# theouterlimitz/Audio-Mastering-Engine

Measured on NVIDIA B200. Metric: audio-sec mastered/sec (x realtime), higher is better.
Workload: dtype f64

## Files before the change

### audio_mastering_engine_b200/csrc/ame.cu

```cuda
#include <algorithm>
#include <cmath>
#include <cstdarg>
#include <cstdio>
#include <cstring>
#include <dlfcn.h>
#include <mutex>
#include <string>
#include <vector>

#include "ame_kernels.cuh"

using namespace ame;

namespace {

thread_local std::string g_err;

int fail(int code, const char *fmt, ...) {
    char buf[512];
    va_list ap;
    va_start(ap, fmt);
    vsnprintf(buf, sizeof buf, fmt, ap);
    va_end(ap);
    g_err = buf;
// ... 129 lines not shown
    int *d_meter_sp = nullptr;
    unsigned *d_meter_tp = nullptr;
    ame_loudness *d_loud_out = nullptr;
    ame_loudness *d_loud_any = nullptr;
    cudaStream_t s_in = nullptr, s_out = nullptr;
    std::vector<cudaEvent_t> ev_in, ev_run;
    std::vector<cudaEvent_t> ev_meter;
    bool timing = false;
    int t_step = -1, t_wave = 0;
    std::vector<cudaEvent_t> t_ev;
    std::vector<char> t_used;
    std::vector<cudaEvent_t> tl_ev;
    int tl_waves = 0;
};

namespace {

inline bool t_on(const ame_plan *p) {
    return p->timing && p->t_step >= 0 && p->t_step < kMaxTimedSteps && p->t_wave < kMaxTimedWaves;
}
inline size_t t_slot(const ame_plan *p, int kernel) {
    return ((size_t)p->t_step * kMaxTimedWaves + p->t_wave) * AME_N_KERNELS + kernel;
}
inline void t_begin(ame_plan *p, int kernel, cudaStream_t s) {
    if (t_on(p)) cudaEventRecord(p->t_ev[t_slot(p, kernel) * 2], s);
}
inline void t_end(ame_plan *p, int kernel, cudaStream_t s) {
    if (t_on(p)) {
        cudaEventRecord(p->t_ev[t_slot(p, kernel) * 2 + 1], s);
        p->t_used[t_slot(p, kernel)] = 1;
    }
}

int plan_alloc(ame_plan *p, void **ptr, size_t bytes) {
    *ptr = nullptr;
    if (bytes == 0) return AME_OK;
    cudaError_t e = dev_alloc(ptr, bytes);
    if (e != cudaSuccess) {
        *ptr = nullptr;
        return fail(AME_E_NOMEM, "device allocation of %zu bytes failed: %s", bytes, cudaGetErrorString(e));
    }
    p->allocs.push_back(*ptr);
    return AME_OK;
}

int dmalloc(ame_plan *p, void **ptr, size_t bytes) {
    const int rc = plan_alloc(p, ptr, bytes);
    if (rc == AME_OK) p->ws_bytes += bytes;
    return rc;
}

template <class T>
int upload(ame_plan *p, T **dptr, const std::vector<T> &v) {
    if (int rc = plan_alloc(p, (void **)dptr, v.size() * sizeof(T))) return rc;
    if (!v.empty()) CU(cudaMemcpy(*dptr, v.data(), v.size() * sizeof(T), cudaMemcpyHostToDevice));
    return AME_OK;
}

#define LAUNCH_CHECK(p)                                                                            \
    do {                                                                                           \
        cudaError_t e_ = cudaGetLastError();                                                       \
        if (e_ != cudaSuccess) return fail(AME_E_CUDA, "kernel launch failed: %s (%s:%d)", cudaGetErrorString(e_), __FILE__, __LINE__); \
        ++(p)->launches;                                                                           \
    } while (0)

int check_warmth(const ame_plan *p) {
    for (int t = 0; t < p->n_tracks; ++t)
        if (p->tracks[t].flags & AME_F_WARMTH) {
            const int l = p->tracks[t].warm_lut;
            if (l < 0 || l >= p->n_luts) return fail(AME_E_INVALID, "track %d needs warmth table %d but %d are set", t, l, p->n_luts);
        }
    return AME_OK;
}

struct Bufs {
    const int16_t *in = nullptr;
    int16_t *pre = nullptr, *bands = nullptr, *out = nullptr;
    uint16_t *rms = nullptr, *list = nullptr;
    int *tile_cnt = nullptr, *n_flagged = nullptr;
    GrpRec *grp = nullptr;
    double *att = nullptr;
    int64_t *hist = nullptr;
    int16_t *norm = nullptr;
    long long *lim_last = nullptr;
    LimStore lim_in{}, lim_out{};
    int *lim_need = nullptr;
};

Bufs slot_bufs(ame_plan *p, const Wave &w, const int16_t *d_in, int16_t *d_out) {
    const Slot &sl = p->slots[w.slot];
    Bufs b;
    b.in = d_in; b.out = d_out;
    b.pre = sl.pre - 2 * w.frame_lo;
    b.bands = sl.bands; b.rms = sl.rms; b.list = sl.list; b.tile_cnt = sl.tile_cnt; b.n_flagged = sl.n_flagged;
    b.grp = sl.grp; b.att = sl.att;
    b.norm = sl.norm ? sl.norm - 2 * w.frame_lo : nullptr;
    b.lim_last = sl.lim_last; b.lim_in = sl.lim_in; b.lim_out = sl.lim_out; b.lim_need = sl.lim_need;
    b.hist = (int64_t *)p->d_hist;
    return b;
}

int run_eq(ame_plan *p, const Wave &w, const int16_t *d_in, int16_t *d_pre, cudaStream_t s) {
    if (!w.eq.n) return AME_OK;
    t_begin(p, S_EQ, s);
    if (p->precision == 1)
        k_eq_f32<<<(w.eq.n + 127) / 128, 128, 0, s>>>(p->d_eq_jobs + w.eq.lo, w.eq.n, p->d_tracks, p->d_luts, d_in, d_pre);
    else
        k_eq<<<(w.eq.n + kEqBlock - 1) / kEqBlock, kEqBlock, 0, s>>>(p->d_eq_jobs + w.eq.lo, w.eq.n, p->d_tracks, p->d_luts, d_in, d_pre);
    LAUNCH_CHECK(p);
    t_end(p, S_EQ, s);
    return AME_OK;
}

int run_split(ame_plan *p, const Wave &w, const int16_t *d_pre, int16_t *d_bands, cudaStream_t s) {
    if (!w.split.n) return AME_OK;
    t_begin(p, S_SPLIT, s);
    if (w.xover_uni)
        k_band_split<true><<<(w.split.n + 127) / 128, 128, 0, s>>>(w.xover, p->d_split_jobs + w.split.lo, w.split.n, p->d_tracks, p->d_mb_delta,
                                                                   d_pre, d_bands, p->mb_frames);
    else
        k_band_split<false><<<(w.split.n + 127) / 128, 128, 0, s>>>(w.xover, p->d_split_jobs + w.split.lo, w.split.n, p->d_tracks, p->d_mb_delta,
                                                                    d_pre, d_bands, p->mb_frames);
    LAUNCH_CHECK(p);
    t_end(p, S_SPLIT, s);
    return AME_OK;
}

int chain_lanes(const ame_plan *p, int n_chains) {
    if (p->chain_warps < 0) return 1;
    if (p->chain_warps > 0) return 32 * p->chain_warps;
    if (n_chains * 2 <= p->n_sm) return 256;
    return (n_chains >= p->n_sm && p->slots.size() > 1) ? 64 : 128;
}

int run_compress(ame_plan *p, const Wave &w, const Bufs &b, cudaStream_t s) {
    if (!w.chain.n) return AME_OK;
    t_begin(p, S_FLAG, s);
    int *tile_base = b.tile_cnt + std::max(p->slot_tiles, 1);
    k_window_flag<<<w.wf.n, kWfThreads, 0, s>>>(p->d_wf_jobs + w.wf.lo, b.bands, b.rms, b.tile_cnt, b.grp);
    LAUNCH_CHECK(p);
    k_tile_prefix<<<w.chain.n, kWfThreads, 0, s>>>(p->d_chain_jobs + w.chain.lo, b.tile_cnt, tile_base, b.n_flagged);
    LAUNCH_CHECK(p);
    k_compact<<<(w.wf.n + kWfThreads / 32 - 1) / (kWfThreads / 32), kWfThreads, 0, s>>>(p->d_wf_jobs + w.wf.lo, w.wf.n, b.rms, b.tile_cnt,
                                                                                          tile_base, b.list, b.grp);
    LAUNCH_CHECK(p);
    t_end(p, S_FLAG, s);
    t_begin(p, S_CHAIN, s);
    const int lanes = chain_lanes(p, w.chain.n);
    k_att_chain<<<w.chain.n, std::max(lanes, 32), 0, s>>>(p->d_chain_jobs + w.chain.lo, b.list, b.n_flagged, p->d_tables, b.att, p->mb_frames,
                                            lanes, p->d_chain_stats + 2 * (size_t)w.chain.lo);
    LAUNCH_CHECK(p);
    t_end(p, S_CHAIN, s);
    t_begin(p, S_APPLY, s);
    k_compress_apply<<<(unsigned)((w.seg_hi - w.seg_lo + 3) / 4), 128, 0, s>>>(p->d_mb_chunks + w.mb_chunks.lo, w.mb_chunks.n, w.seg_lo, w.seg_hi,
                                                                                b.bands, b.grp, b.att, b.pre, p->mb_frames);
    LAUNCH_CHECK(p);
    t_end(p, S_APPLY, s);
    return AME_OK;
}

int run_hist(ame_plan *p, const Wave &w, const int16_t *d_pre, int64_t *d_hist, cudaStream_t s) {
    const int nt = w.track_hi - w.track_lo;
    if (nt <= 0) return AME_OK;
    CU(cudaMemsetAsync(p->d_peak + w.track_lo, 0, (size_t)nt * 4, s));
    if (w.kw.n) {
        t_begin(p, S_KW, s);
        if (w.kw_uni)
            k_kweight_energy<true><<<(w.kw.n + 127) / 128, 128, 0, s>>>(w.kw_cfg, p->d_kw_jobs + w.kw.lo, w.kw.n, p->d_tracks, p->d_tdev, d_pre,
                                                                        p->d_energy, p->d_peak);
        else
            k_kweight_energy<false><<<(w.kw.n + 127) / 128, 128, 0, s>>>(w.kw_cfg, p->d_kw_jobs + w.kw.lo, w.kw.n, p->d_tracks, p->d_tdev, d_pre,
                                                                         p->d_energy, p->d_peak);
        LAUNCH_CHECK(p);
        t_end(p, S_KW, s);
    }
    t_begin(p, S_TAIL, s);
    k_tail_peak<<<nt, 128, 0, s>>>(p->d_tracks, p->d_tdev, w.track_lo, w.track_hi, d_pre, p->d_peak);
    LAUNCH_CHECK(p);
    t_end(p, S_TAIL, s);
    CU(cudaMemsetAsync(p->d_tp + w.track_lo, 0, (size_t)nt * 4, s));
    if (w.true_peak && w.gain.n) {
        t_begin(p, S_TP, s);
        k_true_peak<<<w.gain.n, 256, 0, s>>>(p->d_gain_jobs + w.gain.lo, p->d_tracks, d_pre, p->d_tp);
        LAUNCH_CHECK(p);
        t_end(p, S_TP, s);
    }
    t_begin(p, S_HIST, s);
    k_block_hist<<<nt, 256, 0, s>>>(p->d_tdev, w.track_lo, p->d_energy, (long long *)d_hist, p->d_hist_st);
    LAUNCH_CHECK(p);
    t_end(p, S_HIST, s);
    return AME_OK;
}

int run_apply(ame_plan *p, const Wave &w, const int16_t *d_pre, int16_t *d_out, const Bufs &b, cudaStream_t s) {
    int16_t *d_norm = b.norm;
    long long *lim_last = b.lim_last;
    if (!w.gain.n) return AME_OK;
    t_begin(p, S_GAIN, s);
    if (w.limiter) CU(cudaMemsetAsync(lim_last, 0xff, (size_t)w.lim.n * sizeof(long long), s));
    k_apply_gain<<<w.gain.n, 256, 0, s>>>(p->d_gain_jobs + w.gain.lo, p->d_results, p->d_tracks, p->d_tdev, d_pre, d_out, d_norm, lim_last);
    LAUNCH_CHECK(p);
    t_end(p, S_GAIN, s);
    if (w.limiter) {
        t_begin(p, S_LIM, s);
        const GainJob *gj = p->d_lim_jobs + w.lim.lo;
        constexpr int kLimRounds = 2;
        int cap = 64;
        while (cap < p->lim_keep + 2) cap *= 2;
        const size_t smem = lim_smem_bytes(cap);
        for (int round = 0; round <= kLimRounds; ++round) {
            if (round == 0) {
                k_limiter<<<w.lim.n, 256, smem, s>>>(gj, w.lim.n, lim_last, p->d_tracks, d_norm, d_out, b.lim_in, b.lim_out, b.lim_need, 0, cap, p->lim_guess);
                LAUNCH_CHECK(p);
            }
            k_limiter<<<w.lim.n, 32, smem, s>>>(gj, w.lim.n, lim_last, p->d_tracks, d_norm, d_out, b.lim_in, b.lim_out, b.lim_need, round, cap, p->lim_guess);
            LAUNCH_CHECK(p);
            k_lim_verify<<<(w.lim.n + 3) / 4, 128, 0, s>>>(gj, w.lim.n, p->d_tracks, b.lim_in, b.lim_out, b.lim_need,
                                                             p->d_lim_stats + round);
            LAUNCH_CHECK(p);
        }
        k_lim_fallback<<<w.lim.n, 32, smem, s>>>(gj, w.lim.n, p->d_tracks, d_norm, d_out, b.lim_in, b.lim_out, b.lim_need, cap);
        LAUNCH_CHECK(p);
        t_end(p, S_LIM, s);
    }
    return AME_OK;
}

int run_gain(ame_plan *p, const Wave &w, const int16_t *d_pre, const int64_t *d_hist, int16_t *d_out, const Bufs &b, cudaStream_t s) {
    const int nt = w.track_hi - w.track_lo;
    if (nt <= 0) return AME_OK;
    t_begin(p, S_FIN, s);
    k_finalize<<<nt, 128, 0, s>>>(p->d_tracks, w.track_lo, w.track_hi, (const long long *)d_hist, p->d_hist_st, p->d_peak,
                                             p->d_tp, p->d_results);
    LAUNCH_CHECK(p);
    t_end(p, S_FIN, s);
    return run_apply(p, w, d_pre, d_out, b, s);
}

int run_meter(ame_plan *p, const Wave &w, const int16_t *buf, ame_loudness *res, cudaStream_t s) {
    if (!w.meter_tracks.n) return AME_OK;
    const int nt = w.track_hi - w.track_lo;
    CU(cudaMemsetAsync(p->d_meter_sp + w.track_lo, 0, (size_t)nt * 4, s));
    CU(cudaMemsetAsync(p->d_meter_tp + w.track_lo, 0, (size_t)nt * 4, s));
    if (w.meter_kw.n) {
        if (w.kw_uni)
            k_kweight_energy<true><<<(w.meter_kw.n + 127) / 128, 128, 0, s>>>(w.kw_cfg, p->d_meter_kw + w.meter_kw.lo, w.meter_kw.n, p->d_tracks,
                                                                              p->d_meter_tdev, buf, p->d_meter_energy, p->d_meter_sp);
        else
            k_kweight_energy<false><<<(w.meter_kw.n + 127) / 128, 128, 0, s>>>(w.kw_cfg, p->d_meter_kw + w.meter_kw.lo, w.meter_kw.n, p->d_tracks,
                                                                               p->d_meter_tdev, buf, p->d_meter_energy, p->d_meter_sp);
        LAUNCH_CHECK(p);
    }
    if (w.meter_peak.n) {
        k_meter_peak<<<w.meter_peak.n, 256, 0, s>>>(p->d_meter_peak + w.meter_peak.lo, p->d_tracks, buf, p->d_meter_tp, p->d_meter_sp);
        LAUNCH_CHECK(p);
    }
    k_meter_finalize<<<w.meter_tracks.n, 256, 0, s>>>(p->d_meter_tracks + w.meter_tracks.lo, p->d_tracks, p->d_meter_tdev, p->d_meter_energy,
                                                      p->d_meter_sp, p->d_meter_tp, res);
    LAUNCH_CHECK(p);
    return AME_OK;
}

int run_measure(ame_plan *p, const Wave &w, const Bufs &b, cudaStream_t s) {
    int rc;
    if ((rc = run_eq(p, w, b.in, b.pre, s))) return rc;
    if ((rc = run_split(p, w, b.pre, b.bands, s))) return rc;
    if ((rc = run_compress(p, w, b, s))) return rc;
    return run_hist(p, w, b.pre, b.hist, s);
}

int run_chain_of_stages(ame_plan *p, const Wave &w, const Bufs &b, cudaStream_t s) {
    int rc = run_measure(p, w, b, s);
    if (rc) return rc;
    return run_gain(p, w, b.pre, b.hist, b.out, b, s);
}

int drain(ame_plan *p, int rc) {
    (void)p;
    if (rc != AME_OK) cudaDeviceSynchronize();
    return rc;
}

}

extern "C" {

int ame_abi_version(void) { return AME_ABI_VERSION; }
size_t ame_sizeof_track_params(void) { return sizeof(ame_track_params); }
size_t ame_sizeof_track_result(void) { return sizeof(ame_track_result); }
size_t ame_sizeof_plan_options(void) { return sizeof(ame_plan_options); }
size_t ame_sizeof_loudness(void) { return sizeof(ame_loudness); }
const char *ame_last_error(void) { return g_err.c_str(); }
const char *ame_kernel_name(int slot) { return (slot >= 0 && slot < AME_N_KERNELS) ? kKernelNames[slot] : ""; }

int ame_device_count(int *count) {
    if (!count) return fail(AME_E_INVALID, "count is NULL");
    *count = 0;
    CU(cudaGetDeviceCount(count));
    return AME_OK;
}

void ame_plan_destroy(ame_plan *p) {
    if (!p) return;
    DeviceGuard guard(p->device);
    cudaDeviceSynchronize();
    for (void *q : p->allocs) dev_free(q);
// ... 601 lines not shown
```

### audio_mastering_engine_b200/csrc/ame_kernels.cuh

```cuda
#pragma once
#include <cuda_runtime.h>
#include <stdint.h>
#include "ame_layout.h"

namespace ame {

constexpr unsigned kFull = 0xffffffffu;

__constant__ double c_hist_bounds[1001];
__constant__ double c_hist_energy[1000];

__device__ __forceinline__ uint4 ldg16(const uint4 *p) { return __ldg(p); }

__device__ __forceinline__ double bq_step(const ame_biquad &c, double &z0, double &z1, double x) {
    double y = fma(c.b0, x, z0);
    z0 = fma(-c.a1, y, fma(c.b1, x, z1));
    z1 = fma(-c.a2, y, c.b2 * x);
    return y;
}

__device__ __forceinline__ double i16_to_f64(int x) {
    return __hiloint2double(0x43300000, (int)(0x80000000u ^ (unsigned)x)) - 4503601774854144.0;
}

// ... 507 lines not shown
    int exp0;
    bool open;
    bool ok;
};

__device__ __forceinline__ void segsum_begin(SegSum &u, double start) {
    u.margin = 0x7fffffffffffffffLL; u.at_p = 0; u.lo = 0; u.hi = -1; u.p = 0;
    u.exp0 = (int)(__double_as_longlong(start) >> 52);
    u.open = true; u.ok = u.exp0 > 0;
}

template <bool DUAL>
__device__ __forceinline__ bool list_step8(const AttEntry *e, double *al, int64_t i, int64_t lim, bool avec, double &a, double &b,
                                           SegSum &u, double &max_m, double &sum_dec) {
    double o[8];
#pragma unroll
    for (int k = 0; k < 8; ++k) {
        if (!DUAL) { max_m = fmax(max_m, e[k].m); sum_dec += e[k].dec; }
        if (DUAL && u.open && i + k < lim) {
            const long long ib = __double_as_longlong(b), im = __double_as_longlong(e[k].m);
            if (ib > im) {
                u.margin = min(u.margin, ib - im);
                const long long id = __double_as_longlong(e[k].dec);
                if (id != 0) {
                    const int ed = (int)(id >> 52);
                    const long long mant = (id & 0xfffffffffffffLL) | (ed ? (1LL << 52) : 0LL);
                    if ((ed ? ed : 1) + (__ffsll(mant) - 1) == u.exp0 - 1) u.ok = false;
                }
                ++u.p;
            } else {
                u.open = false;
                u.at_p = ib; u.lo = __double_as_longlong(e[k].tau); u.hi = im;
                if ((int)(ib >> 52) != u.exp0) u.ok = false;
            }
        }
        b = att_update(b, e[k].m, e[k].inc, e[k].dec, e[k].tau);
        if (DUAL) a = att_update(a, e[k].m, e[k].inc, e[k].dec, e[k].tau);
        o[k] = b;
    }
    if (avec && i + 8 <= lim) {
        double2 *d = reinterpret_cast<double2 *>(al + i);
        d[0] = make_double2(o[0], o[1]); d[1] = make_double2(o[2], o[3]);
        d[2] = make_double2(o[4], o[5]); d[3] = make_double2(o[6], o[7]);
    } else {
#pragma unroll
        for (int k = 0; k < 8; ++k)
            if (i + k < lim) al[i + k] = o[k];
    }
    return DUAL && __double_as_longlong(a) == __double_as_longlong(b);
}

template <bool DUAL>
__device__ __forceinline__ bool list_walk(const uint16_t *lp, const AttEntry *tbl, double *al, int64_t b0, int64_t b1, bool vec,
                                          bool avec, double a, double &b, SegSum &u, double &max_m, double &sum_dec) {
    if (b0 >= b1) return false;
    RmsBlk r0 = list_load(lp, b0, b1, vec), r1 = list_load(lp, b0 + 8, b1, vec);
    AttEntry ea[8], eb[8];
    list_entries(ea, tbl, r0);
    for (int64_t i = b0; i < b1; i += 16) {
        r0 = list_load(lp, i + 16, b1, vec);
        list_entries(eb, tbl, r1);
        if (list_step8<DUAL>(ea, al, i, b1, avec, a, b, u, max_m, sum_dec)) return true;
        if (i + 8 >= b1) break;
        r1 = list_load(lp, i + 24, b1, vec);
        list_entries(ea, tbl, r0);
        if (list_step8<DUAL>(eb, al, i + 8, b1, avec, a, b, u, max_m, sum_dec)) return true;
    }
    return false;
}

__global__ void __launch_bounds__(kChainMaxThreads)
k_att_chain(const ChainJob *__restrict__ jobs, const uint16_t *__restrict__ list, const int *__restrict__ n_flagged,
            const AttEntry *__restrict__ tables, double *att, int64_t mb_frames, int n_lanes,
            int *__restrict__ stats) {
    __shared__ double s_end[kChainMaxThreads], s_maxm[kChainMaxThreads], s_dec[kChainMaxThreads], s_guess[kChainMaxThreads];
    const ChainJob job = jobs[blockIdx.x];
    const int t = threadIdx.x;
    const uint16_t *lp = list + (int64_t)job.band * mb_frames + job.mb_begin;
    double *al = att + (int64_t)job.band * mb_frames + job.mb_begin;
    const AttEntry *tbl = tables + (size_t)job.table * 32769;
    const bool vec = (reinterpret_cast<uintptr_t>(lp) & 15) == 0;
    const bool avec = (reinterpret_cast<uintptr_t>(al) & 15) == 0;
    const int64_t n_f = n_flagged[blockIdx.x];

    int S = n_lanes < 1 ? 1 : (n_lanes > (int)blockDim.x ? (int)blockDim.x : n_lanes);
    int64_t seg = (((n_f + S - 1) / S) + 7) & ~(int64_t)7;
    if (seg < 64) seg = 64;
    const int S_used = (int)((n_f + seg - 1) / seg);
    const int64_t b0 = min(n_f, (int64_t)t * seg), b1 = min(n_f, b0 + seg);
    double start = 0.0;
    if (t > 0 && b0 < b1) start = tbl[__ldg(lp + b0 - 1)].m;
    double end = start;
    SegSum u;
    segsum_begin(u, start);
    u.ok = false;
    double max_m = 0.0, sum_dec = 0.0;
    list_walk<false>(lp, tbl, al, b0, b1, vec, avec, 0.0, end, u, max_m, sum_dec);
    s_end[t] = end; s_maxm[t] = max_m; s_dec[t] = sum_dec; s_guess[t] = -1.0;
    __syncthreads();
    if (t == 0) {
        double lb = s_end[0];
        for (int v = 1; v < S_used; ++v) {
            const double lo = lb - 1.000001 * s_dec[v];
            if (lb > 0.0 && lo > s_maxm[v]) { s_guess[v] = lb; lb = lo; }
            else lb = s_end[v];
        }
    }
    __syncthreads();
    long long pending = 0;
    auto flush = [&]() {
        if (pending) {
            for (int64_t i = b0; i < b0 + u.p; ++i) al[i] = __longlong_as_double(__double_as_longlong(al[i]) + pending);
            pending = 0;
        }
    };
    int passes = 1;
    for (;;) {
        s_end[t] = end;
        __syncthreads();
        double from = (t > 0 && t < S_used) ? s_end[t - 1] : 0.0;
        if (passes == 1 && t < S_used && s_guess[t] >= 0.0) from = s_guess[t];
        const bool redo = t < S_used && __double_as_longlong(from) != __double_as_longlong(start);
        const int n_redo = __syncthreads_count(redo);
        if (!n_redo) break;
        ++passes;
        if (redo) {
            const long long fb = __double_as_longlong(from), d = fb - __double_as_longlong(start);
            const bool parked = u.open;
            bool quick = u.ok && (int)(fb >> 52) == u.exp0 && (d >= 0 || u.p == 0 || u.margin > -d);
            if (quick && parked) quick = (int)((__double_as_longlong(end) + d) >> 52) == u.exp0;
            if (quick && !parked) quick = u.at_p >= u.lo && u.at_p <= u.hi && u.at_p + d >= u.lo && u.at_p + d <= u.hi &&
                                          (int)((u.at_p + d) >> 52) == u.exp0;
            if (quick) {
                pending += d;
                if (u.p) u.margin += d;
                if (parked) end = __longlong_as_double(__double_as_longlong(end) + d);
                else u.at_p += d;
                start = from;
            } else {
                flush();
                double b = from;
                segsum_begin(u, from);
                const bool met = list_walk<true>(lp, tbl, al, b0, b1, vec, avec, start, b, u, max_m, sum_dec);
                if (!met) end = b;
                if (u.open && (met || (int)(__double_as_longlong(end) >> 52) != u.exp0)) u.ok = false;
                start = from;
            }
        }
    }
    flush();
    if (stats && t == 0) { stats[2 * blockIdx.x] = (int)min(n_f, (int64_t)0x7fffffff); stats[2 * blockIdx.x + 1] = passes; }
}

__device__ __forceinline__ int mul_floor(int x, double f) {
    return max(__double2int_rd(__dmul_rn((double)x, f)), -32768);
}

__device__ __noinline__ double gain_of_att(double att) { return exp10(-att / 20.0); }

__global__ void __launch_bounds__(128, 5)
k_compress_apply(const MbChunk *__restrict__ chunks, int n_chunks, int64_t seg_lo, int64_t seg_hi,
                 const int16_t *__restrict__ bands, const GrpRec *__restrict__ grp, const double *__restrict__ att,
                 int16_t *__restrict__ pre, int64_t mb_frames) {
    const int64_t seg = seg_lo + (int64_t)blockIdx.x * (blockDim.x >> 5) + (threadIdx.x >> 5);
    if (seg >= seg_hi) return;
    const int lane = threadIdx.x & 31;
    int lo = 0, hi = n_chunks - 1;
    while (lo < hi) {
        const int mid = (lo + hi + 1) >> 1;
        if (chunks[mid].seg_prefix <= seg) lo = mid; else hi = mid - 1;
    }
    const MbChunk ck = chunks[lo];
    const int64_t lseg = seg - ck.seg_prefix;
    const int64_t f0 = lseg * kSeg;
    const int64_t n = ck.n;
    uint32_t wv[3][8];
    GrpRec rec[3][8];
#pragma unroll
    for (int b = 0; b < 3; ++b) {
        const uint32_t *bp = reinterpret_cast<const uint32_t *>(bands) + (int64_t)b * mb_frames + ck.mb_begin;
        const GrpRec *gp = grp + ck.grp_begin[b] + lseg * 8;
#pragma unroll
        for (int g = 0; g < 8; ++g) {
            const int64_t i = f0 + g * 32 + lane;
            wv[b][g] = (i < n) ? __ldg(bp + i) : 0u;
            const uint2 r = (f0 + g * 32 < n) ? __ldg(reinterpret_cast<const uint2 *>(gp + g)) : make_uint2(0u, 0u);
            rec[b][g] = GrpRec{r.x, r.y};
        }
    }
    double av[3][8];
#pragma unroll
    for (int b = 0; b < 3; ++b) {
        const double *ap = att + (int64_t)b * mb_frames + ck.mb_begin;
#pragma unroll
        for (int g = 0; g < 8; ++g) {
            const unsigned rank = rec[b][g].base + __popc(rec[b][g].mask & (0xffffffffu >> (31 - lane)));
            av[b][g] = rank ? __ldg(ap + (rank - 1)) : 0.0;
        }
    }
    int accl[8], accr[8];
#pragma unroll
    for (int b = 0; b < 3; ++b) {
        double c_att = 0.0, c_fac = 1.0;
#pragma unroll
        for (int g = 0; g < 8; ++g) {
            const uint32_t w = wv[b][g];
            int l = (int16_t)(w & 0xffffu), r = (int16_t)(w >> 16);
            const double mine = av[b][g];
            if (mine != 0.0) {
                if (mine != c_att) { c_att = mine; c_fac = gain_of_att(mine); }
                l = mul_floor(l, c_fac);
                r = mul_floor(r, c_fac);
            }
            accl[g] = b ? sat16(accl[g] + l) : l;
            accr[g] = b ? sat16(accr[g] + r) : r;
        }
    }
    uint32_t *out = reinterpret_cast<uint32_t *>(pre) + ck.abs_begin;
#pragma unroll
    for (int g = 0; g < 8; ++g) {
        const int64_t i = f0 + g * 32 + lane;
        if (i < n) out[i] = pack16(accl[g], accr[g]);
    }
}

template <bool UNI>
__global__ void __launch_bounds__(128, 5)
k_kweight_energy(const __grid_constant__ KwCfg kc, const KwJob *__restrict__ jobs, int n_jobs, const ame_track_params *__restrict__ tracks,
                 const TrackDev *__restrict__ tdev, const int16_t *__restrict__ pre,
                 double *__restrict__ energy, int *__restrict__ peak) {
    const int j = blockIdx.x * blockDim.x + threadIdx.x;
    if (j >= n_jobs) return;
    const KwJob job = jobs[j];
    const ame_track_params *tp = tracks + job.track;
    const TrackDev td = tdev[job.track];
    const ame_biquad k0 = UNI ? ame_biquad{kc.b0, kc.b1, kc.b2, kc.a1, kc.a2} : tp->kw[0];
    const ame_biquad k1 = UNI ? ame_biquad{1.0, -2.0, 1.0, kc.ra1, kc.ra2} : tp->kw[1];
    const int64_t s100 = td.s100;
    const int64_t base = tp->offset_frames;
    const int64_t t_begin = (int64_t)job.sb_begin * s100;
    const int64_t t_end = (int64_t)job.sb_end * s100;
    int64_t f_lo = t_begin - (int64_t)tp->warm_kw;
    if (f_lo < 0) f_lo = 0;
    f_lo &= ~(int64_t)7;
    double zl[4] = {0, 0, 0, 0}, zr[4] = {0, 0, 0, 0}, accl = 0, accr = 0;
    int pk = 0;
    int64_t next_end = t_begin + s100;
    int sb = job.sb_begin;
    const uint4 *src = reinterpret_cast<const uint4 *>(reinterpret_cast<const uint32_t *>(pre) + base + f_lo);
    const int n_it = (int)((t_end - f_lo + 7) >> 3);
    uint4 c0 = ldg16(src), c1 = ldg16(src + 1), n0 = c0, n1 = c1;
    if (n_it > 1) { n0 = ldg16(src + 2); n1 = ldg16(src + 3); }
    for (int it = 0; it < n_it; ++it) {
        uint4 m0 = n0, m1 = n1;
        if (it + 2 < n_it) { m0 = ldg16(src + 2 * it + 4); m1 = ldg16(src + 2 * it + 5); }
        const int64_t g = f_lo + 8 * (int64_t)it;
        const uint32_t w[8] = {c0.x, c0.y, c0.z, c0.w, c1.x, c1.y, c1.z, c1.w};
        if (g + 8 <= t_begin) {
#pragma unroll
            for (int k = 0; k < 8; ++k) {
                const int xl = (int)(int16_t)(w[k] & 0xffffu), xr = (int)(int16_t)(w[k] >> 16);
                bq_step(k1, zl[2], zl[3], bq_step(k0, zl[0], zl[1], i16_to_unit(xl)));
                bq_step(k1, zr[2], zr[3], bq_step(k0, zr[0], zr[1], i16_to_unit(xr)));
            }
        } else if (g >= t_begin && g + 8 <= next_end) {
#pragma unroll
            for (int k = 0; k < 8; ++k) {
                const int xl = (int)(int16_t)(w[k] & 0xffffu), xr = (int)(int16_t)(w[k] >> 16);
                const double yl = bq_step(k1, zl[2], zl[3], bq_step(k0, zl[0], zl[1], i16_to_unit(xl)));
                const double yr = bq_step(k1, zr[2], zr[3], bq_step(k0, zr[0], zr[1], i16_to_unit(xr)));
                accl = fma(yl, yl, accl);
                accr = fma(yr, yr, accr);
                pk = max(pk, max(abs(xl), abs(xr)));
            }
            if (g + 8 == next_end) {
                energy[td.sb_offset + sb] = accl + accr;
                accl = 0; accr = 0; ++sb; next_end += s100;
            }
        } else {
#pragma unroll
            for (int k = 0; k < 8; ++k) {
                const int64_t f = g + k;
                const int xl = (int)(int16_t)(w[k] & 0xffffu), xr = (int)(int16_t)(w[k] >> 16);
                const double yl = bq_step(k1, zl[2], zl[3], bq_step(k0, zl[0], zl[1], i16_to_unit(xl)));
                const double yr = bq_step(k1, zr[2], zr[3], bq_step(k0, zr[0], zr[1], i16_to_unit(xr)));
                if (f >= t_begin && f < t_end) {
                    accl = fma(yl, yl, accl);
                    accr = fma(yr, yr, accr);
                    pk = max(pk, max(abs(xl), abs(xr)));
                    if (f + 1 == next_end) {
                        energy[td.sb_offset + sb] = accl + accr;
                        accl = 0; accr = 0; ++sb; next_end += s100;
                    }
                }
            }
        }
        c0 = n0; c1 = n1; n0 = m0; n1 = m1;
    }
    atomicMax(peak + job.track, pk);
}

__global__ void k_tail_peak(const ame_track_params *__restrict__ tracks, const TrackDev *__restrict__ tdev,
                            int track_lo, int track_hi, const int16_t *__restrict__ pre, int *__restrict__ peak) {
    const int t = track_lo + blockIdx.x;
    if (t >= track_hi) return;
    const int64_t begin = (int64_t)tdev[t].n_sb * tdev[t].s100;
    const int16_t *p = pre + 2 * tracks[t].offset_frames;
    int pk = 0;
    for (int64_t i = 2 * begin + threadIdx.x; i < 2 * tdev[t].n_total; i += blockDim.x) pk = max(pk, abs((int)p[i]));
    atomicMax(peak + t, pk);
}

__device__ __forceinline__ int hist_index(double e) {
    int lo = 0, hi = 1000;
    do {
        int mid = (lo + hi) >> 1;
        if (e >= c_hist_bounds[mid]) lo = mid; else hi = mid;
    } while (hi - lo != 1);
    return lo;
}

__global__ void __launch_bounds__(256)
k_block_hist(const TrackDev *__restrict__ tdev, int track_lo, const double *__restrict__ energy, long long *__restrict__ hist,
             int *__restrict__ hist_st) {
    __shared__ unsigned s_hist[1000];
    __shared__ unsigned s_st[1000];
    const int t = track_lo + blockIdx.x;
    for (int i = threadIdx.x; i < 1000; i += blockDim.x) { s_hist[i] = 0; s_st[i] = 0; }
    __syncthreads();
    const TrackDev td = tdev[t];
    const double *e = energy + td.sb_offset;
    const double denom = (double)(4 * (int64_t)td.s100);
    for (int j = td.first_block + threadIdx.x; j + 3 < td.n_sb; j += blockDim.x) {
        const double s = (((e[j] + e[j + 1]) + e[j + 2]) + e[j + 3]) / denom;
        if (s >= c_hist_bounds[0]) atomicAdd(&s_hist[hist_index(s)], 1u);
    }
    const double denom_st = (double)(30 * (int64_t)td.s100);
    for (int k = threadIdx.x; 10 * k + 29 < td.n_sb; k += blockDim.x) {
        double s = 0.0;
        for (int j = 0; j < 30; ++j) s += e[10 * k + j];
        s /= denom_st;
        if (s >= c_hist_bounds[0]) atomicAdd(&s_st[hist_index(s)], 1u);
    }
    __syncthreads();
    for (int i = threadIdx.x; i < 1000; i += blockDim.x) {
        hist[(int64_t)t * 1000 + i] = (long long)s_hist[i];
        hist_st[(int64_t)t * 1000 + i] = (int)s_st[i];
    }
}

struct GateWalk { long long count, above; double rel, thresh, integrated; };
template <class H>
__device__ __forceinline__ GateWalk gate_walk(const H *h) {
    GateWalk g{0, 0, 0.0, -70.0, -INFINITY};
    double rel = 0.0; long long count = 0;
    for (int j = 0; j < 1000; ++j) { rel += (double)h[j] * c_hist_energy[j]; count += h[j]; }
    g.count = count;
    if (count > 0) {
        rel /= (double)count;
        rel *= 0.1;
        g.rel = rel;
        g.thresh = 10.0 * log10(rel) - 0.691;
        int start;
        if (rel < c_hist_bounds[0]) start = 0;
        else { start = hist_index(rel); if (rel > c_hist_energy[start]) ++start; }
        double gated = 0.0; long long above = 0;
        for (int j = start; j < 1000; ++j) { gated += (double)h[j] * c_hist_energy[j]; above += h[j]; }
        g.above = above;
        if (above > 0) {
            gated /= (double)above;
            g.integrated = 10.0 * log10(gated) - 0.691;
        }
    }
    return g;
}

// ... 551 lines not shown
```

Before: 928,500.

## Precompute per-flagged-frame gains in a separate kernel and streamline compress apply

Adds a k_att_gain kernel that converts each flagged attenuation value into a linear gain in place before the apply pass, so exp10 is evaluated once per flagged frame instead of per lane run inside k_compress_apply. The apply kernel now loads group records once per warp and broadcasts them with shuffles. It replaces int-to-double conversion and floor with magic-constant bit tricks applied to unpacked 16-bit halves, and uses predicated inline-PTX loads with bounds computed per segment. The cost is an extra kernel launch plus a full read and write pass over the att buffer, and att is overwritten with gains, which matters if anything later reads it as attenuation. Unflagged samples are now multiplied by 1.0 instead of being skipped.

```diff
diff --git a/audio_mastering_engine_b200/csrc/ame.cu b/audio_mastering_engine_b200/csrc/ame.cu
--- a/audio_mastering_engine_b200/csrc/ame.cu
+++ b/audio_mastering_engine_b200/csrc/ame.cu
@@ -305,6 +305,8 @@
     LAUNCH_CHECK(p);
     t_end(p, S_CHAIN, s);
     t_begin(p, S_APPLY, s);
+    k_att_gain<<<dim3(w.chain.n, kGainSplit), kGainThreads, 0, s>>>(p->d_chain_jobs + w.chain.lo, b.n_flagged, b.att, p->mb_frames);
+    LAUNCH_CHECK(p);
     k_compress_apply<<<(unsigned)((w.seg_hi - w.seg_lo + 3) / 4), 128, 0, s>>>(p->d_mb_chunks + w.mb_chunks.lo, w.mb_chunks.n, w.seg_lo, w.seg_hi,
                                                                                 b.bands, b.grp, b.att, b.pre, p->mb_frames);
     LAUNCH_CHECK(p);
diff --git a/audio_mastering_engine_b200/csrc/ame_kernels.cuh b/audio_mastering_engine_b200/csrc/ame_kernels.cuh
--- a/audio_mastering_engine_b200/csrc/ame_kernels.cuh
+++ b/audio_mastering_engine_b200/csrc/ame_kernels.cuh
@@ -683,15 +683,36 @@
     if (stats && t == 0) { stats[2 * blockIdx.x] = (int)min(n_f, (int64_t)0x7fffffff); stats[2 * blockIdx.x + 1] = passes; }
 }
 
-__device__ __forceinline__ int mul_floor(int x, double f) {
-    return max(__double2int_rd(__dmul_rn((double)x, f)), -32768);
+constexpr int kGainThreads = 256;
+constexpr int kGainSplit = 16;
+constexpr int kApplyCtas = 5;
+
+template <int S>
+__device__ __forceinline__ int mul_floor(uint32_t v, double f) {
+    const double x = __hiloint2double(0x43300000, (int)v) - (S ? 0x1.00000800p52 : 0x1.00000000080p52);
+    return max(__double2loint(__dadd_rd(__dmul_rn(x, f), S ? 0x1.8p68 : 0x1.8p52)), -32768);
 }
 
 __device__ __noinline__ double gain_of_att(double att) { return exp10(-att / 20.0); }
 
-__global__ void __launch_bounds__(128, 5)
+__global__ void __launch_bounds__(kGainThreads)
+k_att_gain(const ChainJob *__restrict__ jobs, const int *__restrict__ n_flagged, double *att, int64_t mb_frames) {
+    const ChainJob job = jobs[blockIdx.x];
+    double *al = att + (int64_t)job.band * mb_frames + job.mb_begin;
+    const int n_f = n_flagged[blockIdx.x];
+    for (int i = blockIdx.y * kGainThreads + threadIdx.x; i < n_f; i += kGainSplit * kGainThreads) al[i] = gain_of_att(al[i]);
+}
+
+__device__ __forceinline__ uint32_t ld_word(const uint32_t *p, bool ok) {
+    uint32_t v;
+    asm volatile("{\n\t.reg .pred q;\n\tsetp.ne.b32 q, %2, 0;\n\tmov.b32 %0, 0;\n\t@q ld.global.nc.u32 %0, [%1];\n\t}"
+                 : "=r"(v) : "l"(p), "r"((int)ok));
+    return v;
+}
+
+__global__ void __launch_bounds__(128, kApplyCtas)
 k_compress_apply(const MbChunk *__restrict__ chunks, int n_chunks, int64_t seg_lo, int64_t seg_hi,
-                 const int16_t *__restrict__ bands, const GrpRec *__restrict__ grp, const double *__restrict__ att,
+                 const int16_t *__restrict__ bands, const GrpRec *__restrict__ grp, const double *__restrict__ gain,
                  int16_t *__restrict__ pre, int64_t mb_frames) {
     const int64_t seg = seg_lo + (int64_t)blockIdx.x * (blockDim.x >> 5) + (threadIdx.x >> 5);
     if (seg >= seg_hi) return;
@@ -704,55 +725,48 @@
     const MbChunk ck = chunks[lo];
     const int64_t lseg = seg - ck.seg_prefix;
     const int64_t f0 = lseg * kSeg;
-    const int64_t n = ck.n;
+    const int left = (int)min(ck.n - f0, (int64_t)kSeg);
+    const unsigned upto = 0xffffffffu >> (31 - lane);
+    uint2 rec = make_uint2(0u, 0u);
+    {
+        const int b = lane >> 3, g = lane & 7;
+        const int64_t gb = b == 0 ? ck.grp_begin[0] : (b == 1 ? ck.grp_begin[1] : ck.grp_begin[2]);
+        if (lane < 24 && g * 32 < left) rec = __ldg(reinterpret_cast<const uint2 *>(grp + gb + lseg * 8 + g));
+    }
     uint32_t wv[3][8];
-    GrpRec rec[3][8];
 #pragma unroll
     for (int b = 0; b < 3; ++b) {
-        const uint32_t *bp = reinterpret_cast<const uint32_t *>(bands) + (int64_t)b * mb_frames + ck.mb_begin;
-        const GrpRec *gp = grp + ck.grp_begin[b] + lseg * 8;
+        const uint32_t *bp = reinterpret_cast<const uint32_t *>(bands) + (int64_t)b * mb_frames + ck.mb_begin + f0 + lane;
+#pragma unroll
+        for (int g = 0; g < 8; ++g) wv[b][g] = ld_word(bp + g * 32, g * 32 + lane < left);
+    }
+    double gv[3][8];
+#pragma unroll
+    for (int b = 0; b < 3; ++b) {
+        const double *ap = gain + (int64_t)b * mb_frames + ck.mb_begin - 1;
 #pragma unroll
         for (int g = 0; g < 8; ++g) {
-            const int64_t i = f0 + g * 32 + lane;
-            wv[b][g] = (i < n) ? __ldg(bp + i) : 0u;
-            const uint2 r = (f0 + g * 32 < n) ? __ldg(reinterpret_cast<const uint2 *>(gp + g)) : make_uint2(0u, 0u);
-            rec[b][g] = GrpRec{r.x, r.y};
-        }
-    }
-    double av[3][8];
+            const unsigned mask = __shfl_sync(kFull, rec.x, b * 8 + g), base = __shfl_sync(kFull, rec.y, b * 8 + g);
+            const unsigned rank = base + __popc(mask & upto);
+            gv[b][g] = rank ? __ldg(ap + rank) : 1.0;
+        }
+    }
+    int accl[8], accr[8];
 #pragma unroll
     for (int b = 0; b < 3; ++b) {
-        const double *ap = att + (int64_t)b * mb_frames + ck.mb_begin;
 #pragma unroll
         for (int g = 0; g < 8; ++g) {
-            const unsigned rank = rec[b][g].base + __popc(rec[b][g].mask & (0xffffffffu >> (31 - lane)));
-            av[b][g] = rank ? __ldg(ap + (rank - 1)) : 0.0;
-        }
-    }
-    int accl[8], accr[8];
-#pragma unroll
-    for (int b = 0; b < 3; ++b) {
-        double c_att = 0.0, c_fac = 1.0;
-#pragma unroll
-        for (int g = 0; g < 8; ++g) {
-            const uint32_t w = wv[b][g];
-            int l = (int16_t)(w & 0xffffu), r = (int16_t)(w >> 16);
-            const double mine = av[b][g];
-            if (mine != 0.0) {
-                if (mine != c_att) { c_att = mine; c_fac = gain_of_att(mine); }
-                l = mul_floor(l, c_fac);
-                r = mul_floor(r, c_fac);
-            }
+            const uint32_t u = wv[b][g] ^ 0x80008000u;
+            const int l = mul_floor<0>(u & 0xffffu, gv[b][g]);
+            const int r = mul_floor<16>(u & 0xffff0000u, gv[b][g]);
             accl[g] = b ? sat16(accl[g] + l) : l;
             accr[g] = b ? sat16(accr[g] + r) : r;
         }
     }
-    uint32_t *out = reinterpret_cast<uint32_t *>(pre) + ck.abs_begin;
-#pragma unroll
-    for (int g = 0; g < 8; ++g) {
-        const int64_t i = f0 + g * 32 + lane;
-        if (i < n) out[i] = pack16(accl[g], accr[g]);
-    }
+    uint32_t *out = reinterpret_cast<uint32_t *>(pre) + ck.abs_begin + f0 + lane;
+#pragma unroll
+    for (int g = 0; g < 8; ++g)
+        if (g * 32 + lane < left) out[g * 32] = pack16(accl[g], accr[g]);
 }
 
 template <bool UNI>
```

New measurement: 949,000 (median of 6 runs). 2.2% higher.
